# PKU-DAIR/Hetu-Galvatron

Measured on NVIDIA H100. Metric: tokens/sec Llama-3.2-1B-shaped ZeRO-2 training step at 1/2/4/8 H100 vs ref CPU, higher is better.
Workload: dtype bf16

## Files before the change

### hetu-galvatron_b200/csrc/bg_gemm.cu

```cuda
#include <stdlib.h>

#include "bg_ctx.cuh"

using namespace bg;

namespace {

constexpr int BLOCK_M = 128, BLOCK_N = 128, BLOCK_K = 64, WGMMA_K = 16;
constexpr int kStages = 5;
constexpr int kABytes = BLOCK_M * BLOCK_K * 2, kBBytes = BLOCK_N * BLOCK_K * 2, kStageBytes = kABytes + kBBytes;
constexpr int kStoreCols = 64;
constexpr int kStoreBytes = BLOCK_M * kStoreCols * 2;
constexpr int kNumStoreBufs = 2;
constexpr int kSmemBytes = kStages * kStageBytes + kNumStoreBufs * kStoreBytes + 1024  + 256 ;
constexpr int kEpiThreads = 256, kThreads = kEpiThreads + 32;
constexpr int kProducerWarp = kEpiThreads / 32;
constexpr int kMaxRegs = 136;
constexpr int kWgOffset = 8192;
constexpr int kGroupM = 16;
static_assert(kSmemBytes <= 227 * 1024, "H100: at most 227 KiB of shared memory per block");
static_assert(kThreads * kMaxRegs + 3 * 128 * 64 <= 65536, "a GEMM CTA and three slim collective CTAs share an SM's registers");
static_assert(kSmemBytes + 1024 + 3 * 1024 <= 228 * 1024, "a GEMM CTA and three slim collective CTAs share an SM's shared memory");

enum Layout { kTN = 0, kNN = 1, kNT = 2 };

__device__ __forceinline__ uint32_t smem_u32(const void* p) { return (uint32_t)__cvta_generic_to_shared(p); }

__device__ __forceinline__ void mbar_init(uint32_t bar, uint32_t count) {
    asm volatile("mbarrier.init.shared::cta.b64 [%0], %1;" ::"r"(bar), "r"(count));
}
__device__ __forceinline__ void mbar_wait(uint32_t bar, uint32_t parity) {
    asm volatile(
        "{\n\t.reg .pred p;\n\t"
        "WAIT_%=:\n\t"
        "mbarrier.try_wait.parity.shared::cta.b64 p, [%0], %1;\n\t"
        "@p bra DONE_%=;\n\t"
        "bra WAIT_%=;\n\t"
        "DONE_%=:\n\t}" ::"r"(bar), "r"(parity) : "memory");
}
__device__ __forceinline__ void mbar_arrive(uint32_t bar) {
    asm volatile("mbarrier.arrive.shared::cta.b64 _, [%0];" ::"r"(bar) : "memory");
}
__device__ __forceinline__ void mbar_expect_tx(uint32_t bar, uint32_t bytes) {
    asm volatile("mbarrier.arrive.expect_tx.shared::cta.b64 _, [%0], %1;" ::"r"(bar), "r"(bytes) : "memory");
}
__device__ __forceinline__ void tma_load_2d(uint32_t dst, const CUtensorMap* map, uint32_t bar, int c0, int c1) {
    asm volatile("cp.async.bulk.tensor.2d.shared::cluster.global.mbarrier::complete_tx::bytes [%0], [%1, {%3, %4}], [%2];"
                 ::"r"(dst), "l"(map), "r"(bar), "r"(c0), "r"(c1) : "memory");
}
__device__ __forceinline__ void tma_store_2d(const CUtensorMap* map, uint32_t src, int c0, int c1) {
    asm volatile("cp.async.bulk.tensor.2d.global.shared::cta.bulk_group [%0, {%2, %3}], [%1];"
                 ::"l"(map), "r"(src), "r"(c0), "r"(c1) : "memory");
}
__device__ __forceinline__ void tma_store_commit() { asm volatile("cp.async.bulk.commit_group;" ::: "memory"); }
template <int N>
__device__ __forceinline__ void tma_store_wait_read() { asm volatile("cp.async.bulk.wait_group.read %0;" ::"n"(N) : "memory"); }
template <int N>
__device__ __forceinline__ void tma_store_wait_all() { asm volatile("cp.async.bulk.wait_group %0;" ::"n"(N) : "memory"); }
__device__ __forceinline__ void fence_proxy_async() { asm volatile("fence.proxy.async.shared::cta;" ::: "memory"); }
__device__ __forceinline__ void epi_bar_sync() { asm volatile("bar.sync 1, %0;" ::"n"(kEpiThreads) : "memory"); }
__device__ __forceinline__ bool elect_one() {
    uint32_t pred;
    asm volatile("{\n\t.reg .pred p;\n\telect.sync _|p, 0xffffffff;\n\tselp.u32 %0, 1, 0, p;\n\t}" : "=r"(pred));
    return pred != 0;
}

__device__ __forceinline__ void wgmma_fence() { asm volatile("wgmma.fence.sync.aligned;" ::: "memory"); }
__device__ __forceinline__ void wgmma_commit() { asm volatile("wgmma.commit_group.sync.aligned;" ::: "memory"); }
template <int N>
__device__ __forceinline__ void wgmma_wait() { asm volatile("wgmma.wait_group.sync.aligned %0;" ::"n"(N) : "memory"); }
__device__ __forceinline__ void fence_acc(float* d) {
#pragma unroll
    for (int i = 0; i < BLOCK_N / 2; ++i) asm volatile("" : "+f"(d[i])::"memory");
}

template <int kTransA, int kTransB>
__device__ __forceinline__ void wgmma_m64n128(float* d, uint64_t desc_a, uint64_t desc_b, uint32_t accumulate) {
    asm volatile(
        "{\n\t.reg .pred p;\n\t"
        "setp.ne.b32 p, %66, 0;\n\t"
        "wgmma.mma_async.sync.aligned.m64n128k16.f32.bf16.bf16 "
        "{%0, %1, %2, %3, %4, %5, %6, %7, %8, %9, %10, %11, %12, %13, %14, %15, "
        "%16, %17, %18, %19, %20, %21, %22, %23, %24, %25, %26, %27, %28, %29, %30, %31, "
        "%32, %33, %34, %35, %36, %37, %38, %39, %40, %41, %42, %43, %44, %45, %46, %47, "
        "%48, %49, %50, %51, %52, %53, %54, %55, %56, %57, %58, %59, %60, %61, %62, %63}, "
        "%64, %65, p, 1, 1, %67, %68;\n\t}"
        : "+f"(d[0]), "+f"(d[1]), "+f"(d[2]), "+f"(d[3]), "+f"(d[4]), "+f"(d[5]), "+f"(d[6]), "+f"(d[7]),
          "+f"(d[8]), "+f"(d[9]), "+f"(d[10]), "+f"(d[11]), "+f"(d[12]), "+f"(d[13]), "+f"(d[14]), "+f"(d[15]),
          "+f"(d[16]), "+f"(d[17]), "+f"(d[18]), "+f"(d[19]), "+f"(d[20]), "+f"(d[21]), "+f"(d[22]), "+f"(d[23]),
          "+f"(d[24]), "+f"(d[25]), "+f"(d[26]), "+f"(d[27]), "+f"(d[28]), "+f"(d[29]), "+f"(d[30]), "+f"(d[31]),
          "+f"(d[32]), "+f"(d[33]), "+f"(d[34]), "+f"(d[35]), "+f"(d[36]), "+f"(d[37]), "+f"(d[38]), "+f"(d[39]),
          "+f"(d[40]), "+f"(d[41]), "+f"(d[42]), "+f"(d[43]), "+f"(d[44]), "+f"(d[45]), "+f"(d[46]), "+f"(d[47]),
          "+f"(d[48]), "+f"(d[49]), "+f"(d[50]), "+f"(d[51]), "+f"(d[52]), "+f"(d[53]), "+f"(d[54]), "+f"(d[55]),
          "+f"(d[56]), "+f"(d[57]), "+f"(d[58]), "+f"(d[59]), "+f"(d[60]), "+f"(d[61]), "+f"(d[62]), "+f"(d[63])
        : "l"(desc_a), "l"(desc_b), "r"(accumulate), "n"(kTransA), "n"(kTransB));
}

__device__ __forceinline__ uint64_t make_smem_desc(uint32_t smem_addr, uint32_t lbo_bytes, uint32_t sbo_bytes) {
    uint64_t d = 0;
    d |= (uint64_t)((smem_addr >> 4) & 0x3fff);
    d |= (uint64_t)((lbo_bytes >> 4) & 0x3fff) << 16;
    d |= (uint64_t)((sbo_bytes >> 4) & 0x3fff) << 32;
    d |= (uint64_t)1 << 62;
    return d;
}

struct TileCoord { int m, n; };
enum { kPlain = 0, kScatterMode = 1, kGatherMode = 2 };

template <int kMode>
struct FuseParams {};

template <>
struct FuseParams<kPlain> {
    int group_m;
};

__device__ __forceinline__ TileCoord tile_of_virtual(int t, int m_blocks, int n_blocks, int group_m) {
    const int per_group = group_m * n_blocks;
    const int g = t / per_group, first_m = g * group_m;
    const int rows = min(group_m, m_blocks - first_m);
    const int r = t - g * per_group;
    return {first_m + r % rows, r / rows};
}

template <>
struct FuseParams<kScatterMode> {
    CUtensorMap dst[BG_MAX_PEERS];
    uint32_t* flags[BG_MAX_PEERS];
    int p, me, rows_per_rank;
};

template <>
struct FuseParams<kGatherMode> {
    CUtensorMap a_local;
    const uint32_t* flags;
    uint32_t target;
    int p, me, blocks_per_rank;
    unsigned long long timeout_ns;
    int* err;
};

template <int kMode>
__device__ __forceinline__ int map_m(int mv, int m_blocks, const FuseParams<kMode>& fp) {
    if constexpr (kMode == kScatterMode) {
        int m = mv + ((fp.me + 1) % fp.p) * (fp.rows_per_rank / BLOCK_M);
        return m >= m_blocks ? m - m_blocks : m;
    } else if constexpr (kMode == kGatherMode) {
        const int c = mv / fp.p, k = mv - c * fp.p;
        int slot = fp.me + k; if (slot >= fp.p) slot -= fp.p;
        return slot * fp.blocks_per_rank + c;
    } else {
        return mv;
    }
}
template <int kMode>
__device__ __forceinline__ TileCoord tile_of(int t, int m_blocks, int n_blocks, const FuseParams<kMode>& fp) {
    int group_m = kGroupM;
    if constexpr (kMode == kPlain) group_m = fp.group_m;
    TileCoord tc = tile_of_virtual(t, m_blocks, n_blocks, group_m);
    tc.m = map_m<kMode>(tc.m, m_blocks, fp);
    return tc;
}

template <int kLayout, int kMode = kPlain>
__global__ void __maxnreg__(kMaxRegs) gemm_bf16_kernel(const __grid_constant__ CUtensorMap map_a,
                                                                const __grid_constant__ CUtensorMap map_b,
                                                                const __grid_constant__ CUtensorMap map_c,
                                                                const __nv_bfloat16* __restrict__ c_old, int M, int N, int K,
                                                                int accumulate,
                                                                const __grid_constant__ FuseParams<kMode> sp) {
    constexpr bool kScatter = kMode == kScatterMode, kGather = kMode == kGatherMode;
    constexpr bool kAMn = kLayout == kNT, kBMn = kLayout != kTN;
    extern __shared__ uint8_t smem_raw[];
    uint8_t* smem = reinterpret_cast<uint8_t*>((reinterpret_cast<uintptr_t>(smem_raw) + 1023) & ~uintptr_t(1023));
    uint8_t* smem_store = smem + kStages * kStageBytes;
    uint64_t* bars = reinterpret_cast<uint64_t*>(smem_store + kNumStoreBufs * kStoreBytes);
    uint64_t* full_bar = bars;
    uint64_t* empty_bar = bars + kStages;

    const int warp = threadIdx.x >> 5, lane = threadIdx.x & 31;
    const int m_blocks = (M + BLOCK_M - 1) / BLOCK_M, n_blocks = (N + BLOCK_N - 1) / BLOCK_N;
    const int num_tiles = m_blocks * n_blocks, k_blocks = (K + BLOCK_K - 1) / BLOCK_K;

    if constexpr (kScatter) {
        asm volatile("griddepcontrol.launch_dependents;" ::: "memory");
    }
    if (warp == kProducerWarp && lane == 0) {
        asm volatile("prefetch.tensormap [%0];" ::"l"(&map_a) : "memory");
        asm volatile("prefetch.tensormap [%0];" ::"l"(&map_b) : "memory");
        asm volatile("prefetch.tensormap [%0];" ::"l"(&map_c) : "memory");
        for (int i = 0; i < kStages; ++i) { mbar_init(smem_u32(full_bar + i), 1); mbar_init(smem_u32(empty_bar + i), kEpiThreads / 32); }
        asm volatile("fence.mbarrier_init.release.cluster;" ::: "memory");
    }
    __syncthreads();

    if (warp == kProducerWarp) {
        if (elect_one()) {
            int stage = 0; uint32_t phase = 0;
            for (int t = blockIdx.x; t < num_tiles; t += gridDim.x) {
                const TileCoord tc = tile_of<kMode>(t, m_blocks, n_blocks, sp);
                const CUtensorMap* amap = &map_a;
                int a_row = tc.m * BLOCK_M;
                if constexpr (kGather) {
                    const int slot = tc.m / sp.blocks_per_rank, c = tc.m - slot * sp.blocks_per_rank;
                    if (slot == sp.me) {
                        amap = &sp.a_local; a_row = c * BLOCK_M;
                    } else {
                        const uint32_t* f = sp.flags + slot * sp.blocks_per_rank + c;
                        unsigned long long t0 = 0; unsigned spins = 0;
                        while (true) {
                            uint32_t v;
                            asm volatile("ld.acquire.sys.global.u32 %0, [%1];" : "=r"(v) : "l"(f) : "memory");
                            if (v >= sp.target) break;
                            if ((++spins & 0x3ff) == 0) {
                                unsigned long long now = gtimer();
                                if (t0 == 0) t0 = now;
                                else if (now - t0 > sp.timeout_ns) {
                                    if (atomicCAS(sp.err + 1, 0, 4) == 0) { sp.err[2] = (int)blockIdx.x; sp.err[3] = tc.m; sp.err[4] = (int)v; sp.err[5] = (int)sp.target; sp.err[6] = slot; }
                                    *sp.err = BG_ETIMEOUT; __threadfence_system(); __trap();
                                }
                            }
                        }
                        asm volatile("fence.proxy.async.global;" ::: "memory");
                    }
                }
                for (int kb = 0; kb < k_blocks; ++kb) {
                    mbar_wait(smem_u32(empty_bar + stage), phase ^ 1);
                    const uint32_t bar = smem_u32(full_bar + stage);
                    const uint32_t sa = smem_u32(smem + stage * kStageBytes), sb = sa + kABytes;
                    mbar_expect_tx(bar, kStageBytes);
                    if (kAMn) {
#pragma unroll
                        for (int j = 0; j < BLOCK_M / 64; ++j) tma_load_2d(sa + j * (BLOCK_K * 128), &map_a, bar, tc.m * BLOCK_M + j * 64, kb * BLOCK_K);
                    } else {
                        tma_load_2d(sa, amap, bar, kb * BLOCK_K, a_row);
                    }
                    if (kBMn) {
#pragma unroll
                        for (int j = 0; j < BLOCK_N / 64; ++j) tma_load_2d(sb + j * (BLOCK_K * 128), &map_b, bar, tc.n * BLOCK_N + j * 64, kb * BLOCK_K);
                    } else {
                        tma_load_2d(sb, &map_b, bar, kb * BLOCK_K, tc.n * BLOCK_N);
                    }
                    if (++stage == kStages) { stage = 0; phase ^= 1; }
                }
            }
        }
    } else {
        const int wg = warp >> 2;
        const int frag_row = wg * 64 + (warp & 3) * 16 + (lane >> 2);
        const int frag_col = (lane & 3) * 2;
        const bool issuer = threadIdx.x == 0;
        constexpr uint32_t a_lbo = kAMn ? BLOCK_K * 128 : 0, b_lbo = kBMn ? BLOCK_K * 128 : 0;
        constexpr uint32_t a_kstep = kAMn ? WGMMA_K * 128 : WGMMA_K * 2, b_kstep = kBMn ? WGMMA_K * 128 : WGMMA_K * 2;
        float acc[BLOCK_N / 2];
#pragma unroll
        for (int i = 0; i < BLOCK_N / 2; ++i) acc[i] = 0.f;
        int stage = 0; uint32_t phase = 0;
        int buf = 0;
        uint32_t* prev_flag = nullptr;
        for (int t = blockIdx.x; t < num_tiles; t += gridDim.x) {
            const TileCoord tc = tile_of<kMode>(t, m_blocks, n_blocks, sp);
            int prev_stage = 0;
            for (int kb = 0; kb < k_blocks; ++kb) {
                mbar_wait(smem_u32(full_bar + stage), phase);
                const uint32_t sa = smem_u32(smem + stage * kStageBytes) + wg * kWgOffset;
                const uint32_t sb = smem_u32(smem + stage * kStageBytes) + kABytes;
                wgmma_fence();
#pragma unroll
                for (int k = 0; k < BLOCK_K / WGMMA_K; ++k) {
                    const uint64_t da = make_smem_desc(sa + k * a_kstep, a_lbo, 1024);
                    const uint64_t db = make_smem_desc(sb + k * b_kstep, b_lbo, 1024);
                    wgmma_m64n128<kAMn ? 1 : 0, kBMn ? 1 : 0>(acc, da, db, (kb | k) != 0);
                }
                wgmma_commit();
                wgmma_wait<1>();
                if (kb > 0 && lane == 0) mbar_arrive(smem_u32(empty_bar + prev_stage));
                prev_stage = stage;
                if (++stage == kStages) { stage = 0; phase ^= 1; }
            }
            wgmma_wait<0>();
            fence_acc(acc);
            if (lane == 0) mbar_arrive(smem_u32(empty_bar + prev_stage));
#pragma unroll
            for (int c = 0; c < BLOCK_N / kStoreCols; ++c) {
                const int n0 = tc.n * BLOCK_N + c * kStoreCols;
                if (n0 >= N) break;
                float* v = acc + c * (kStoreCols / 2);
                if (accumulate) {
#pragma unroll
                    for (int h = 0; h < 2; ++h) {
                        const long long grow = (long long)tc.m * BLOCK_M + frag_row + 8 * h;
                        if (grow < M) {
#pragma unroll
                            for (int j = 0; j < 8; ++j) {
                                if (n0 + j * 8 < N) {
                                    const float2 o = bf2_to_f2(*reinterpret_cast<const uint32_t*>(c_old + grow * N + n0 + j * 8 + frag_col));
                                    v[j * 4 + 2 * h] += o.x;
                                    v[j * 4 + 2 * h + 1] += o.y;
                                }
                            }
                        }
                    }
                }
                if (issuer) tma_store_wait_read<kNumStoreBufs - 1>();
                epi_bar_sync();
                uint8_t* sbuf = smem_store + buf * kStoreBytes;
#pragma unroll
                for (int h = 0; h < 2; ++h) {
                    const int row = frag_row + 8 * h;
#pragma unroll
                    for (int j = 0; j < 8; ++j)
                        *reinterpret_cast<uint32_t*>(sbuf + row * 128 + ((j ^ (row & 7)) << 4) + frag_col * 2) =
                            f2_to_bf2(v[j * 4 + 2 * h], v[j * 4 + 2 * h + 1]);
                }
                fence_proxy_async();
                epi_bar_sync();
                if (issuer) {
                    if constexpr (kScatter) {
                        const int row0 = tc.m * BLOCK_M, owner = row0 / sp.rows_per_rank;
                        tma_store_2d(&sp.dst[owner], smem_u32(sbuf), n0, sp.me * sp.rows_per_rank + (row0 - owner * sp.rows_per_rank));
                    } else {
                        tma_store_2d(&map_c, smem_u32(sbuf), n0, tc.m * BLOCK_M);
                    }
                    tma_store_commit();
                }
                buf ^= 1;
            }
            if constexpr (kScatter) {
                if (issuer) {
                    if (prev_flag != nullptr) {
                        asm volatile("cp.async.bulk.wait_group %0;" ::"n"(BLOCK_N / kStoreCols) : "memory");
                        __threadfence_system();
                        asm volatile("red.release.sys.global.add.u32 [%0], 1;" ::"l"(prev_flag) : "memory");
                    }
                    const int row0 = tc.m * BLOCK_M, owner = row0 / sp.rows_per_rank;
                    prev_flag = sp.flags[owner] + ((row0 - owner * sp.rows_per_rank) / BLOCK_M) * n_blocks + tc.n;
                }
            }
        }
        if (issuer) {
            tma_store_wait_all<0>();
            if constexpr (kScatter) {
                if (prev_flag != nullptr) {
                    __threadfence_system();
                    asm volatile("red.release.sys.global.add.u32 [%0], 1;" ::"l"(prev_flag) : "memory");
                }
            }
        }
    }
}

typedef CUresult (*EncodeTiledFn)(CUtensorMap*, CUtensorMapDataType, cuuint32_t, void*, const cuuint64_t*, const cuuint64_t*,
                                  const cuuint32_t*, const cuuint32_t*, CUtensorMapInterleave, CUtensorMapSwizzle,
                                  CUtensorMapL2promotion, CUtensorMapFloatOOBfill);

EncodeTiledFn encode_fn() {
    static EncodeTiledFn fn = nullptr;
    static std::once_flag once;
    std::call_once(once, [] {
        void* p = nullptr;
        cudaDriverEntryPointQueryResult q;
        if (cudaGetDriverEntryPoint("cuTensorMapEncodeTiled", &p, cudaEnableDefault, &q) == cudaSuccess && q == cudaDriverEntryPointSuccess)
            fn = (EncodeTiledFn)p;
    });
    return fn;
}

int make_map(CUtensorMap* map, const void* ptr, long long rows, long long cols, int box_cols, int box_rows) {
    EncodeTiledFn fn = encode_fn();
    if (!fn) return fail(BG_ECUDA, "cuTensorMapEncodeTiled entry point not available");
    cuuint64_t dims[2] = {(cuuint64_t)cols, (cuuint64_t)rows};
    cuuint64_t strides[1] = {(cuuint64_t)cols * 2};
    cuuint32_t box[2] = {(cuuint32_t)box_cols, (cuuint32_t)box_rows};
    cuuint32_t estr[2] = {1, 1};
    CUresult r = fn(map, CU_TENSOR_MAP_DATA_TYPE_BFLOAT16, 2, const_cast<void*>(ptr), dims, strides, box, estr,
                    CU_TENSOR_MAP_INTERLEAVE_NONE, CU_TENSOR_MAP_SWIZZLE_128B, CU_TENSOR_MAP_L2_PROMOTION_L2_256B,
                    CU_TENSOR_MAP_FLOAT_OOB_FILL_NONE);
    if (r == CUDA_ERROR_INVALID_CONTEXT) {
        cudaFree(0);
        r = fn(map, CU_TENSOR_MAP_DATA_TYPE_BFLOAT16, 2, const_cast<void*>(ptr), dims, strides, box, estr,
               CU_TENSOR_MAP_INTERLEAVE_NONE, CU_TENSOR_MAP_SWIZZLE_128B, CU_TENSOR_MAP_L2_PROMOTION_L2_256B,
               CU_TENSOR_MAP_FLOAT_OOB_FILL_NONE);
    }
    if (r != CUDA_SUCCESS) return fail(BG_ECUDA, "cuTensorMapEncodeTiled failed (%d) rows=%lld cols=%lld", (int)r, rows, cols);
    return BG_OK;
}

int g_num_sms = 0;

}

int bg_preload_gemm();

static int gemm_setup() {
    if (g_num_sms == 0) {
        int dev = 0;
        BG_CUDA(cudaGetDevice(&dev));
        int sms = 0;
        BG_CUDA(cudaDeviceGetAttribute(&sms, cudaDevAttrMultiProcessorCount, dev));
#define BG_SMEM(K) BG_CUDA(cudaFuncSetAttribute(K, cudaFuncAttributeMaxDynamicSharedMemorySize, kSmemBytes))
        BG_SMEM(gemm_bf16_kernel<kTN>); BG_SMEM(gemm_bf16_kernel<kNN>); BG_SMEM(gemm_bf16_kernel<kNT>);
        BG_SMEM((gemm_bf16_kernel<kTN, kScatterMode>)); BG_SMEM((gemm_bf16_kernel<kNN, kScatterMode>)); BG_SMEM((gemm_bf16_kernel<kNT, kScatterMode>));
        BG_SMEM((gemm_bf16_kernel<kTN, kGatherMode>)); BG_SMEM((gemm_bf16_kernel<kNN, kGatherMode>));
#undef BG_SMEM
        g_num_sms = sms;
    }
    return BG_OK;
}



static int make_ab_maps(CUtensorMap* ma, CUtensorMap* mb, const void* a, const void* b, long long m, long long n, long long k, int layout) {
    int rc = layout == kNT ? make_map(ma, a, k, m, 64, BLOCK_K) : make_map(ma, a, m, k, BLOCK_K, BLOCK_M);
    if (rc) return rc;
    return layout == kTN ? make_map(mb, b, n, k, BLOCK_K, BLOCK_N) : make_map(mb, b, k, n, 64, BLOCK_K);
}

static int gemm_launch(const void* a, const void* b, void* c, const void* addend, long long m, long long n, long long k, int layout, void* stream);

extern "C" int bg_gemm_bf16(const void* a, const void* b, void* c, long long m, long long n, long long k, int layout,
                            int accumulate, void* stream) {
    return gemm_launch(a, b, c, accumulate ? c : nullptr, m, n, k, layout, stream);
}

extern "C" int bg_gemm_bf16_add(const void* a, const void* b, void* c, const void* addend, long long m, long long n, long long k,
                                int layout, void* stream) {
    if (addend == nullptr || (uintptr_t)addend % 16) return fail(BG_EINVAL, "bg_gemm_bf16_add: addend must be a 16-B aligned [M][N] bf16 tensor");
    return gemm_launch(a, b, c, addend, m, n, k, layout, stream);
}

static int gemm_launch(const void* a, const void* b, void* c, const void* addend, long long m, long long n, long long k, int layout, void* stream) {
    const int accumulate = addend != nullptr;
    if (layout < 0 || layout > 2) return fail(BG_EINVAL, "bg_gemm_bf16: layout %d", layout);
    if (m <= 0 || n <= 0 || k <= 0 || m % 8 || n % 8 || k % 8)
        return fail(BG_EINVAL, "bg_gemm_bf16: m,n,k (%lld,%lld,%lld) must be positive multiples of 8", m, n, k);
    if (((uintptr_t)a | (uintptr_t)b | (uintptr_t)c) % 16) return fail(BG_EINVAL, "bg_gemm_bf16: pointers must be 16-B aligned");
    CUtensorMap ma, mb, mc;
    int rc = make_ab_maps(&ma, &mb, a, b, m, n, k, layout);
    if (rc) return rc;
    rc = make_map(&mc, c, m, n, kStoreCols, BLOCK_M);
    if (rc) return rc;
    rc = gemm_setup();
    if (rc) return rc;
    const long long n_blocks = (n + BLOCK_N - 1) / BLOCK_N, tiles = ((m + BLOCK_M - 1) / BLOCK_M) * n_blocks;
    const int grid = (int)(tiles < g_num_sms ? tiles : g_num_sms);
    cudaStream_t st = (cudaStream_t)stream;
    const __nv_bfloat16* c_old = (const __nv_bfloat16*)addend;
    FuseParams<kPlain> plain;
    plain.group_m = n_blocks <= 32 ? 2 : 8;
    if (layout == kTN) gemm_bf16_kernel<kTN><<<grid, kThreads, kSmemBytes, st>>>(ma, mb, mc, c_old, (int)m, (int)n, (int)k, accumulate, plain);
    else if (layout == kNN) gemm_bf16_kernel<kNN><<<grid, kThreads, kSmemBytes, st>>>(ma, mb, mc, c_old, (int)m, (int)n, (int)k, accumulate, plain);
    else gemm_bf16_kernel<kNT><<<grid, kThreads, kSmemBytes, st>>>(ma, mb, mc, c_old, (int)m, (int)n, (int)k, accumulate, plain);
    BG_CHECK_LAUNCH();
    return BG_OK;
}

namespace {

struct Bcast {
    char* out[BG_MAX_PEERS];
    char* mc;
    int on;
};

__device__ __forceinline__ void mm_st_16g(void* mc, const uint4& v) {
    asm volatile("multimem.st.relaxed.sys.global.v4.f32 [%0], {%1,%2,%3,%4};" ::"l"(mc), "f"(__uint_as_float(v.x)),
                 "f"(__uint_as_float(v.y)), "f"(__uint_as_float(v.z)), "f"(__uint_as_float(v.w)) : "memory");
}

__global__ void __launch_bounds__(128, 8) tile_reduce_kernel(const __nv_bfloat16* __restrict__ partial, uint32_t* __restrict__ flags,
                                                          __nv_bfloat16* __restrict__ out, int p, int me, int rows_per_rank, int N,
                                                          int n_blocks, int local_tiles, const __grid_constant__ Bcast bc,
                                                          unsigned long long timeout_ns, int* err) {
    for (int lt = blockIdx.x; lt < local_tiles; lt += gridDim.x) {
        if (threadIdx.x == 0) {
            unsigned long long t0 = 0;
            unsigned spins = 0;
            while (true) {
                uint32_t v;
                asm volatile("ld.acquire.sys.global.u32 %0, [%1];" : "=r"(v) : "l"(flags + lt) : "memory");
                if (v >= (uint32_t)p) break;
                if ((++spins & 0x3ff) == 0) {
                    unsigned long long now = gtimer();
                    if (t0 == 0) t0 = now;
                    else if (now - t0 > timeout_ns / 2) {
                        if (atomicCAS(err + 1, 0, 3) == 0) { err[2] = (int)blockIdx.x; err[3] = lt; err[4] = (int)v; err[5] = p; err[6] = local_tiles; }
                        *err = BG_ETIMEOUT; __threadfence_system(); __trap();
                    }
                }
            }
        }
        __syncthreads();
        const int mb = lt / n_blocks, nb = lt % n_blocks;
        const int row0 = mb * BLOCK_M, col0 = nb * BLOCK_N;
        const int cols = min(BLOCK_N, N - col0), rows = min(BLOCK_M, rows_per_rank - row0);
        const int vec_per_row = cols / 8;
        for (int i = threadIdx.x; i < rows * vec_per_row; i += blockDim.x) {
            const int r = i / vec_per_row, c = i - r * vec_per_row;
            const size_t off = (size_t)(row0 + r) * N + col0 + c * 8;
            uint4 in[BG_MAX_PEERS];
#pragma unroll
            for (int src = 0; src < BG_MAX_PEERS; ++src)
                if (src < p) in[src] = ld16_stream(partial + (size_t)src * rows_per_rank * N + off);
            float acc[8];
#pragma unroll
            for (int e = 0; e < 8; ++e) acc[e] = 0.f;
#pragma unroll
            for (int src = 0; src < BG_MAX_PEERS; ++src)
                if (src < p) {
                    float f[8];
                    unpack8(in[src], f);
#pragma unroll
                    for (int e = 0; e < 8; ++e) acc[e] += f[e];
                }
            const uint4 o = pack8(acc);
            if (bc.on) {
                const size_t goff = ((size_t)me * rows_per_rank * N + off) * 2;
                if (bc.mc != nullptr) {
                    mm_st_16g(bc.mc + goff, o);
                } else {
                    for (int k = 0; k < p; ++k) {
                        int q = me + k; if (q >= p) q -= p;
                        st16(bc.out[q] + goff, o);
                    }
                }
            } else {
                st16(out + off, o);
            }
        }
        __syncthreads();
        if (threadIdx.x == 0) flags[lt] = 0;
    }
    asm volatile("griddepcontrol.wait;" ::: "memory");
}

}

int bg_gemm_scatter_launch(const void* a, const void* b, long long m, long long n, long long k, int layout, int p, int me,
                           void* const* partial_ptrs, uint32_t* const* flag_ptrs, void* out, void* const* bcast_ptrs, char* bcast_mc,
                           unsigned long long timeout_ns, int* err_dev, cudaStream_t st) {
    if (layout < 0 || layout > 2) return fail(BG_EINVAL, "bg_gemm_reduce_scatter: layout %d", layout);
    if (m <= 0 || n <= 0 || k <= 0 || n % 8 || k % 8) return fail(BG_EINVAL, "bg_gemm_reduce_scatter: bad dims");
    if (m % ((long long)p * BLOCK_M)) return fail(BG_EINVAL, "bg_gemm_reduce_scatter: M=%lld must be a multiple of p*%d", m, BLOCK_M);
    const int rows_per_rank = (int)(m / p);
    CUtensorMap ma, mb;
    int rc = make_ab_maps(&ma, &mb, a, b, m, n, k, layout);
    if (rc) return rc;
    FuseParams<kScatterMode> sp;
    sp.p = p; sp.me = me; sp.rows_per_rank = rows_per_rank;
    for (int i = 0; i < BG_MAX_PEERS; ++i) {
        sp.flags[i] = i < p ? flag_ptrs[i] : nullptr;
        if (i < p) { rc = make_map(&sp.dst[i], partial_ptrs[i], (long long)p * rows_per_rank, n, kStoreCols, BLOCK_M); if (rc) return rc; }
        else sp.dst[i] = sp.dst[0];
    }
    rc = gemm_setup();
    if (rc) return rc;
    const int m_blocks = (int)((m + BLOCK_M - 1) / BLOCK_M), n_blocks = (int)((n + BLOCK_N - 1) / BLOCK_N);
    const long long tiles = (long long)m_blocks * n_blocks;
    const int grid = (int)(tiles < g_num_sms ? tiles : g_num_sms);
    const int local_tiles = (rows_per_rank / BLOCK_M) * n_blocks;
    const CUtensorMap& mc_unused = sp.dst[0];
    if (layout == kTN) gemm_bf16_kernel<kTN, kScatterMode><<<grid, kThreads, kSmemBytes, st>>>(ma, mb, mc_unused, nullptr, (int)m, (int)n, (int)k, 0, sp);
    else if (layout == kNN) gemm_bf16_kernel<kNN, kScatterMode><<<grid, kThreads, kSmemBytes, st>>>(ma, mb, mc_unused, nullptr, (int)m, (int)n, (int)k, 0, sp);
    else gemm_bf16_kernel<kNT, kScatterMode><<<grid, kThreads, kSmemBytes, st>>>(ma, mb, mc_unused, nullptr, (int)m, (int)n, (int)k, 0, sp);
    BG_CHECK_LAUNCH();
    const int rgrid = local_tiles < g_num_sms ? local_tiles : g_num_sms;
    Bcast bc = {};
    if (bcast_ptrs != nullptr) {
        bc.on = 1; bc.mc = bcast_mc;
        for (int i = 0; i < p; ++i) bc.out[i] = (char*)bcast_ptrs[i];
    }
    cudaLaunchConfig_t cfg = {};
    cfg.gridDim = dim3((unsigned)rgrid); cfg.blockDim = dim3(128);
    cudaLaunchAttribute attr[1];
    attr[0].id = cudaLaunchAttributeProgrammaticStreamSerialization;
    attr[0].val.programmaticStreamSerializationAllowed = 1;
    static const bool no_pdl = getenv("HGB_NO_PDL") != nullptr;
    cfg.attrs = attr; cfg.numAttrs = no_pdl ? 0 : 1;
    BG_CUDA(cudaLaunchKernelEx(&cfg, tile_reduce_kernel, (const __nv_bfloat16*)partial_ptrs[me], (uint32_t*)flag_ptrs[me],
                               (__nv_bfloat16*)out, p, me, rows_per_rank, (int)n, n_blocks, local_tiles, bc, timeout_ns, err_dev));
    bg::g_launches.fetch_add(1, std::memory_order_relaxed);
    return BG_OK;
}

int bg_gemm_gather_launch(const void* a_local, const void* a_staged, const void* b, void* c, long long m, long long n, long long k,
                          int layout, int p, int me, const uint32_t* flags, uint32_t target, unsigned long long timeout_ns, int* err_dev,
                          cudaStream_t st) {
    if (layout != kTN && layout != kNN) return fail(BG_EINVAL, "bg_all_gather_gemm: layout %d", layout);
    if (((uintptr_t)a_local | (uintptr_t)a_staged | (uintptr_t)b | (uintptr_t)c) % 16) return fail(BG_EINVAL, "bg_all_gather_gemm: pointers must be 16-B aligned");
    CUtensorMap ma, mb, mc;
    int rc = make_ab_maps(&ma, &mb, a_staged, b, m, n, k, layout);
    if (rc) return rc;
    rc = make_map(&mc, c, m, n, kStoreCols, BLOCK_M);
    if (rc) return rc;
    FuseParams<kGatherMode> gp;
    rc = make_map(&gp.a_local, a_local, m / p, k, BLOCK_K, BLOCK_M);
    if (rc) return rc;
    gp.flags = flags; gp.target = target; gp.p = p; gp.me = me; gp.blocks_per_rank = (int)(m / p / BLOCK_M);
    gp.timeout_ns = timeout_ns; gp.err = err_dev;
    rc = gemm_setup();
    if (rc) return rc;
    const long long tiles = (m / BLOCK_M) * ((n + BLOCK_N - 1) / BLOCK_N);
    const int grid = (int)(tiles < g_num_sms ? tiles : g_num_sms);
    if (layout == kTN) gemm_bf16_kernel<kTN, kGatherMode><<<grid, kThreads, kSmemBytes, st>>>(ma, mb, mc, nullptr, (int)m, (int)n, (int)k, 0, gp);
    else gemm_bf16_kernel<kNN, kGatherMode><<<grid, kThreads, kSmemBytes, st>>>(ma, mb, mc, nullptr, (int)m, (int)n, (int)k, 0, gp);
    BG_CHECK_LAUNCH();
    return BG_OK;
}

int bg_preload_gemm() {
    int rc = gemm_setup();
    if (rc) return rc;
    cudaFuncAttributes attr;
    BG_CUDA(cudaFuncGetAttributes(&attr, reinterpret_cast<const void*>(&tile_reduce_kernel)));
    return BG_OK;
}
```

Baseline: 51740.

## Add 128x256 wide-tile WGMMA path for plain GEMMs with N above 128

Templates the GEMM kernel on tile width and adds a 128x256 variant using m64n256 WGMMA, with 4 stages, a single store buffer and a 168-register cap. Plain GEMMs with N>128 now use the wide tile, which halves B-operand reloads per output and amortizes A loads over twice the columns. The group_m swizzle heuristic also changes. Risks are higher register pressure, fewer pipeline stages, a serialized epilogue store buffer, and fewer tiles, which can leave SMs idle on small GEMMs.

After: 54300 (median of 6 runs). +5.0%, better.

```diff
diff --git a/hetu-galvatron_b200/csrc/bg_gemm.cu b/hetu-galvatron_b200/csrc/bg_gemm.cu
--- a/hetu-galvatron_b200/csrc/bg_gemm.cu
+++ b/hetu-galvatron_b200/csrc/bg_gemm.cu
@@ -7,20 +7,31 @@
 namespace {
 
 constexpr int BLOCK_M = 128, BLOCK_N = 128, BLOCK_K = 64, WGMMA_K = 16;
-constexpr int kStages = 5;
-constexpr int kABytes = BLOCK_M * BLOCK_K * 2, kBBytes = BLOCK_N * BLOCK_K * 2, kStageBytes = kABytes + kBBytes;
+constexpr int WIDE_N = 256;
+constexpr int kABytes = BLOCK_M * BLOCK_K * 2;
 constexpr int kStoreCols = 64;
 constexpr int kStoreBytes = BLOCK_M * kStoreCols * 2;
-constexpr int kNumStoreBufs = 2;
-constexpr int kSmemBytes = kStages * kStageBytes + kNumStoreBufs * kStoreBytes + 1024  + 256 ;
 constexpr int kEpiThreads = 256, kThreads = kEpiThreads + 32;
 constexpr int kProducerWarp = kEpiThreads / 32;
-constexpr int kMaxRegs = 136;
 constexpr int kWgOffset = 8192;
 constexpr int kGroupM = 16;
-static_assert(kSmemBytes <= 227 * 1024, "H100: at most 227 KiB of shared memory per block");
-static_assert(kThreads * kMaxRegs + 3 * 128 * 64 <= 65536, "a GEMM CTA and three slim collective CTAs share an SM's registers");
-static_assert(kSmemBytes + 1024 + 3 * 1024 <= 228 * 1024, "a GEMM CTA and three slim collective CTAs share an SM's shared memory");
+
+template <int kBlockN>
+struct Tile {
+    static constexpr bool kWide = kBlockN == WIDE_N;
+    static constexpr int kStages = kWide ? 4 : 5;
+    static constexpr int kNumStoreBufs = kWide ? 1 : 2;
+    static constexpr int kMaxRegs = kWide ? 168 : 136;
+    static constexpr int kSlimCtas = kWide ? 2 : 3;
+    static constexpr int kBBytes = kBlockN * BLOCK_K * 2, kStageBytes = kABytes + kBBytes;
+    static constexpr int kSmemBytes = kStages * kStageBytes + kNumStoreBufs * kStoreBytes + 1024  + 256 ;
+    static_assert(kBlockN == BLOCK_N || kBlockN == WIDE_N, "tile width 128 or 256");
+    static_assert(kSmemBytes <= 227 * 1024, "H100: at most 227 KiB of shared memory per block");
+    static_assert(kThreads * kMaxRegs + kSlimCtas * 128 * 64 <= 65536, "a GEMM CTA and its slim collective CTAs share an SM's registers");
+    static_assert(kSmemBytes + 1024 + kSlimCtas * 1024 <= 228 * 1024, "a GEMM CTA and its slim collective CTAs share an SM's shared memory");
+};
+template struct Tile<BLOCK_N>;
+template struct Tile<WIDE_N>;
 
 enum Layout { kTN = 0, kNN = 1, kNT = 2 };
 
@@ -69,9 +80,10 @@
 __device__ __forceinline__ void wgmma_commit() { asm volatile("wgmma.commit_group.sync.aligned;" ::: "memory"); }
 template <int N>
 __device__ __forceinline__ void wgmma_wait() { asm volatile("wgmma.wait_group.sync.aligned %0;" ::"n"(N) : "memory"); }
+template <int kNumAcc>
 __device__ __forceinline__ void fence_acc(float* d) {
 #pragma unroll
-    for (int i = 0; i < BLOCK_N / 2; ++i) asm volatile("" : "+f"(d[i])::"memory");
+    for (int i = 0; i < kNumAcc; ++i) asm volatile("" : "+f"(d[i])::"memory");
 }
 
 template <int kTransA, int kTransB>
@@ -96,6 +108,40 @@
         : "l"(desc_a), "l"(desc_b), "r"(accumulate), "n"(kTransA), "n"(kTransB));
 }
 
+template <int kTransA, int kTransB>
+__device__ __forceinline__ void wgmma_m64n256(float* d, uint64_t desc_a, uint64_t desc_b, uint32_t accumulate) {
+    asm volatile(
+        "{\n\t.reg .pred p;\n\t"
+        "setp.ne.b32 p, %130, 0;\n\t"
+        "wgmma.mma_async.sync.aligned.m64n256k16.f32.bf16.bf16 "
+        "{%0, %1, %2, %3, %4, %5, %6, %7, %8, %9, %10, %11, %12, %13, %14, %15, "
+        "%16, %17, %18, %19, %20, %21, %22, %23, %24, %25, %26, %27, %28, %29, %30, %31, "
+        "%32, %33, %34, %35, %36, %37, %38, %39, %40, %41, %42, %43, %44, %45, %46, %47, "
+        "%48, %49, %50, %51, %52, %53, %54, %55, %56, %57, %58, %59, %60, %61, %62, %63, "
+        "%64, %65, %66, %67, %68, %69, %70, %71, %72, %73, %74, %75, %76, %77, %78, %79, "
+        "%80, %81, %82, %83, %84, %85, %86, %87, %88, %89, %90, %91, %92, %93, %94, %95, "
+        "%96, %97, %98, %99, %100, %101, %102, %103, %104, %105, %106, %107, %108, %109, %110, %111, "
+        "%112, %113, %114, %115, %116, %117, %118, %119, %120, %121, %122, %123, %124, %125, %126, %127}, "
+        "%128, %129, p, 1, 1, %131, %132;\n\t}"
+        : "+f"(d[0]), "+f"(d[1]), "+f"(d[2]), "+f"(d[3]), "+f"(d[4]), "+f"(d[5]), "+f"(d[6]), "+f"(d[7]),
+          "+f"(d[8]), "+f"(d[9]), "+f"(d[10]), "+f"(d[11]), "+f"(d[12]), "+f"(d[13]), "+f"(d[14]), "+f"(d[15]),
+          "+f"(d[16]), "+f"(d[17]), "+f"(d[18]), "+f"(d[19]), "+f"(d[20]), "+f"(d[21]), "+f"(d[22]), "+f"(d[23]),
+          "+f"(d[24]), "+f"(d[25]), "+f"(d[26]), "+f"(d[27]), "+f"(d[28]), "+f"(d[29]), "+f"(d[30]), "+f"(d[31]),
+          "+f"(d[32]), "+f"(d[33]), "+f"(d[34]), "+f"(d[35]), "+f"(d[36]), "+f"(d[37]), "+f"(d[38]), "+f"(d[39]),
+          "+f"(d[40]), "+f"(d[41]), "+f"(d[42]), "+f"(d[43]), "+f"(d[44]), "+f"(d[45]), "+f"(d[46]), "+f"(d[47]),
+          "+f"(d[48]), "+f"(d[49]), "+f"(d[50]), "+f"(d[51]), "+f"(d[52]), "+f"(d[53]), "+f"(d[54]), "+f"(d[55]),
+          "+f"(d[56]), "+f"(d[57]), "+f"(d[58]), "+f"(d[59]), "+f"(d[60]), "+f"(d[61]), "+f"(d[62]), "+f"(d[63]),
+          "+f"(d[64]), "+f"(d[65]), "+f"(d[66]), "+f"(d[67]), "+f"(d[68]), "+f"(d[69]), "+f"(d[70]), "+f"(d[71]),
+          "+f"(d[72]), "+f"(d[73]), "+f"(d[74]), "+f"(d[75]), "+f"(d[76]), "+f"(d[77]), "+f"(d[78]), "+f"(d[79]),
+          "+f"(d[80]), "+f"(d[81]), "+f"(d[82]), "+f"(d[83]), "+f"(d[84]), "+f"(d[85]), "+f"(d[86]), "+f"(d[87]),
+          "+f"(d[88]), "+f"(d[89]), "+f"(d[90]), "+f"(d[91]), "+f"(d[92]), "+f"(d[93]), "+f"(d[94]), "+f"(d[95]),
+          "+f"(d[96]), "+f"(d[97]), "+f"(d[98]), "+f"(d[99]), "+f"(d[100]), "+f"(d[101]), "+f"(d[102]), "+f"(d[103]),
+          "+f"(d[104]), "+f"(d[105]), "+f"(d[106]), "+f"(d[107]), "+f"(d[108]), "+f"(d[109]), "+f"(d[110]), "+f"(d[111]),
+          "+f"(d[112]), "+f"(d[113]), "+f"(d[114]), "+f"(d[115]), "+f"(d[116]), "+f"(d[117]), "+f"(d[118]), "+f"(d[119]),
+          "+f"(d[120]), "+f"(d[121]), "+f"(d[122]), "+f"(d[123]), "+f"(d[124]), "+f"(d[125]), "+f"(d[126]), "+f"(d[127])
+        : "l"(desc_a), "l"(desc_b), "r"(accumulate), "n"(kTransA), "n"(kTransB));
+}
+
 __device__ __forceinline__ uint64_t make_smem_desc(uint32_t smem_addr, uint32_t lbo_bytes, uint32_t sbo_bytes) {
     uint64_t d = 0;
     d |= (uint64_t)((smem_addr >> 4) & 0x3fff);
@@ -163,15 +209,18 @@
     return tc;
 }
 
-template <int kLayout, int kMode = kPlain>
-__global__ void __maxnreg__(kMaxRegs) gemm_bf16_kernel(const __grid_constant__ CUtensorMap map_a,
+template <int kLayout, int kMode = kPlain, int kBlockN = BLOCK_N>
+__global__ void __maxnreg__(Tile<kBlockN>::kMaxRegs) gemm_bf16_kernel(const __grid_constant__ CUtensorMap map_a,
                                                                 const __grid_constant__ CUtensorMap map_b,
                                                                 const __grid_constant__ CUtensorMap map_c,
                                                                 const __nv_bfloat16* __restrict__ c_old, int M, int N, int K,
                                                                 int accumulate,
                                                                 const __grid_constant__ FuseParams<kMode> sp) {
+    static_assert(kMode == kPlain || kBlockN == BLOCK_N, "the fused modes wait on peers: they keep the three-slim-CTA tile");
     constexpr bool kScatter = kMode == kScatterMode, kGather = kMode == kGatherMode;
     constexpr bool kAMn = kLayout == kNT, kBMn = kLayout != kTN;
+    constexpr int kStages = Tile<kBlockN>::kStages, kStageBytes = Tile<kBlockN>::kStageBytes;
+    constexpr int kNumStoreBufs = Tile<kBlockN>::kNumStoreBufs;
     extern __shared__ uint8_t smem_raw[];
     uint8_t* smem = reinterpret_cast<uint8_t*>((reinterpret_cast<uintptr_t>(smem_raw) + 1023) & ~uintptr_t(1023));
     uint8_t* smem_store = smem + kStages * kStageBytes;
@@ -180,7 +229,7 @@
     uint64_t* empty_bar = bars + kStages;
 
     const int warp = threadIdx.x >> 5, lane = threadIdx.x & 31;
-    const int m_blocks = (M + BLOCK_M - 1) / BLOCK_M, n_blocks = (N + BLOCK_N - 1) / BLOCK_N;
+    const int m_blocks = (M + BLOCK_M - 1) / BLOCK_M, n_blocks = (N + kBlockN - 1) / kBlockN;
     const int num_tiles = m_blocks * n_blocks, k_blocks = (K + BLOCK_K - 1) / BLOCK_K;
 
     if constexpr (kScatter) {
@@ -238,9 +287,9 @@
                     }
                     if (kBMn) {
 #pragma unroll
-                        for (int j = 0; j < BLOCK_N / 64; ++j) tma_load_2d(sb + j * (BLOCK_K * 128), &map_b, bar, tc.n * BLOCK_N + j * 64, kb * BLOCK_K);
+                        for (int j = 0; j < kBlockN / 64; ++j) tma_load_2d(sb + j * (BLOCK_K * 128), &map_b, bar, tc.n * kBlockN + j * 64, kb * BLOCK_K);
                     } else {
-                        tma_load_2d(sb, &map_b, bar, kb * BLOCK_K, tc.n * BLOCK_N);
+                        tma_load_2d(sb, &map_b, bar, kb * BLOCK_K, tc.n * kBlockN);
                     }
                     if (++stage == kStages) { stage = 0; phase ^= 1; }
                 }
@@ -253,9 +302,9 @@
         const bool issuer = threadIdx.x == 0;
         constexpr uint32_t a_lbo = kAMn ? BLOCK_K * 128 : 0, b_lbo = kBMn ? BLOCK_K * 128 : 0;
         constexpr uint32_t a_kstep = kAMn ? WGMMA_K * 128 : WGMMA_K * 2, b_kstep = kBMn ? WGMMA_K * 128 : WGMMA_K * 2;
-        float acc[BLOCK_N / 2];
-#pragma unroll
-        for (int i = 0; i < BLOCK_N / 2; ++i) acc[i] = 0.f;
+        float acc[kBlockN / 2];
+#pragma unroll
+        for (int i = 0; i < kBlockN / 2; ++i) acc[i] = 0.f;
         int stage = 0; uint32_t phase = 0;
         int buf = 0;
         uint32_t* prev_flag = nullptr;
@@ -271,7 +320,8 @@
                 for (int k = 0; k < BLOCK_K / WGMMA_K; ++k) {
                     const uint64_t da = make_smem_desc(sa + k * a_kstep, a_lbo, 1024);
                     const uint64_t db = make_smem_desc(sb + k * b_kstep, b_lbo, 1024);
-                    wgmma_m64n128<kAMn ? 1 : 0, kBMn ? 1 : 0>(acc, da, db, (kb | k) != 0);
+                    if constexpr (kBlockN == WIDE_N) wgmma_m64n256<kAMn ? 1 : 0, kBMn ? 1 : 0>(acc, da, db, (kb | k) != 0);
+                    else wgmma_m64n128<kAMn ? 1 : 0, kBMn ? 1 : 0>(acc, da, db, (kb | k) != 0);
                 }
                 wgmma_commit();
                 wgmma_wait<1>();
@@ -280,14 +330,30 @@
                 if (++stage == kStages) { stage = 0; phase ^= 1; }
             }
             wgmma_wait<0>();
-            fence_acc(acc);
+            fence_acc<kBlockN / 2>(acc);
             if (lane == 0) mbar_arrive(smem_u32(empty_bar + prev_stage));
 #pragma unroll
-            for (int c = 0; c < BLOCK_N / kStoreCols; ++c) {
-                const int n0 = tc.n * BLOCK_N + c * kStoreCols;
+            for (int c = 0; c < kBlockN / kStoreCols; ++c) {
+                const int n0 = tc.n * kBlockN + c * kStoreCols;
                 if (n0 >= N) break;
                 float* v = acc + c * (kStoreCols / 2);
-                if (accumulate) {
+                if (accumulate && Tile<kBlockN>::kWide) {
+#pragma unroll
+                    for (int h = 0; h < 2; ++h) {
+                        const int grow = tc.m * BLOCK_M + frag_row + 8 * h;
+                        if (grow < M) {
+                            const uint32_t* src = reinterpret_cast<const uint32_t*>(c_old + (long long)grow * N + n0 + frag_col);
+#pragma unroll
+                            for (int j = 0; j < 8; ++j) {
+                                if (n0 + j * 8 < N) {
+                                    const float2 o = bf2_to_f2(src[j * 4]);
+                                    v[j * 4 + 2 * h] += o.x;
+                                    v[j * 4 + 2 * h + 1] += o.y;
+                                }
+                            }
+                        }
+                    }
+                } else if (accumulate) {
 #pragma unroll
                     for (int h = 0; h < 2; ++h) {
                         const long long grow = (long long)tc.m * BLOCK_M + frag_row + 8 * h;
@@ -306,13 +372,25 @@
                 if (issuer) tma_store_wait_read<kNumStoreBufs - 1>();
                 epi_bar_sync();
                 uint8_t* sbuf = smem_store + buf * kStoreBytes;
-#pragma unroll
-                for (int h = 0; h < 2; ++h) {
-                    const int row = frag_row + 8 * h;
-#pragma unroll
-                    for (int j = 0; j < 8; ++j)
-                        *reinterpret_cast<uint32_t*>(sbuf + row * 128 + ((j ^ (row & 7)) << 4) + frag_col * 2) =
-                            f2_to_bf2(v[j * 4 + 2 * h], v[j * 4 + 2 * h + 1]);
+                if constexpr (Tile<kBlockN>::kWide) {
+                    uint32_t srow = smem_u32(sbuf) + frag_row * 128 + ((frag_row & 7) << 4) + frag_col * 2;
+                    asm volatile("" : "+r"(srow));
+#pragma unroll
+                    for (int h = 0; h < 2; ++h) {
+#pragma unroll
+                        for (int j = 0; j < 8; ++j)
+                            asm volatile("st.shared.u32 [%0], %1;" ::"r"((srow + h * 1024) ^ (j << 4)),
+                                         "r"(f2_to_bf2(v[j * 4 + 2 * h], v[j * 4 + 2 * h + 1])) : "memory");
+                    }
+                } else {
+#pragma unroll
+                    for (int h = 0; h < 2; ++h) {
+                        const int row = frag_row + 8 * h;
+#pragma unroll
+                        for (int j = 0; j < 8; ++j)
+                            *reinterpret_cast<uint32_t*>(sbuf + row * 128 + ((j ^ (row & 7)) << 4) + frag_col * 2) =
+                                f2_to_bf2(v[j * 4 + 2 * h], v[j * 4 + 2 * h + 1]);
+                    }
                 }
                 fence_proxy_async();
                 epi_bar_sync();
@@ -325,12 +403,12 @@
                     }
                     tma_store_commit();
                 }
-                buf ^= 1;
+                if constexpr (kNumStoreBufs > 1) buf ^= 1;
             }
             if constexpr (kScatter) {
                 if (issuer) {
                     if (prev_flag != nullptr) {
-                        asm volatile("cp.async.bulk.wait_group %0;" ::"n"(BLOCK_N / kStoreCols) : "memory");
+                        asm volatile("cp.async.bulk.wait_group %0;" ::"n"(kBlockN / kStoreCols) : "memory");
                         __threadfence_system();
                         asm volatile("red.release.sys.global.add.u32 [%0], 1;" ::"l"(prev_flag) : "memory");
                     }
@@ -399,10 +477,13 @@
         BG_CUDA(cudaGetDevice(&dev));
         int sms = 0;
         BG_CUDA(cudaDeviceGetAttribute(&sms, cudaDevAttrMultiProcessorCount, dev));
-#define BG_SMEM(K) BG_CUDA(cudaFuncSetAttribute(K, cudaFuncAttributeMaxDynamicSharedMemorySize, kSmemBytes))
-        BG_SMEM(gemm_bf16_kernel<kTN>); BG_SMEM(gemm_bf16_kernel<kNN>); BG_SMEM(gemm_bf16_kernel<kNT>);
-        BG_SMEM((gemm_bf16_kernel<kTN, kScatterMode>)); BG_SMEM((gemm_bf16_kernel<kNN, kScatterMode>)); BG_SMEM((gemm_bf16_kernel<kNT, kScatterMode>));
-        BG_SMEM((gemm_bf16_kernel<kTN, kGatherMode>)); BG_SMEM((gemm_bf16_kernel<kNN, kGatherMode>));
+#define BG_SMEM(K, W) BG_CUDA(cudaFuncSetAttribute(K, cudaFuncAttributeMaxDynamicSharedMemorySize, Tile<W>::kSmemBytes))
+        BG_SMEM(gemm_bf16_kernel<kTN>, BLOCK_N); BG_SMEM(gemm_bf16_kernel<kNN>, BLOCK_N); BG_SMEM(gemm_bf16_kernel<kNT>, BLOCK_N);
+        BG_SMEM((gemm_bf16_kernel<kTN, kPlain, WIDE_N>), WIDE_N); BG_SMEM((gemm_bf16_kernel<kNN, kPlain, WIDE_N>), WIDE_N);
+        BG_SMEM((gemm_bf16_kernel<kNT, kPlain, WIDE_N>), WIDE_N);
+        BG_SMEM((gemm_bf16_kernel<kTN, kScatterMode>), BLOCK_N); BG_SMEM((gemm_bf16_kernel<kNN, kScatterMode>), BLOCK_N);
+        BG_SMEM((gemm_bf16_kernel<kNT, kScatterMode>), BLOCK_N);
+        BG_SMEM((gemm_bf16_kernel<kTN, kGatherMode>), BLOCK_N); BG_SMEM((gemm_bf16_kernel<kNN, kGatherMode>), BLOCK_N);
 #undef BG_SMEM
         g_num_sms = sms;
     }
@@ -411,10 +492,11 @@
 
 
 
-static int make_ab_maps(CUtensorMap* ma, CUtensorMap* mb, const void* a, const void* b, long long m, long long n, long long k, int layout) {
+static int make_ab_maps(CUtensorMap* ma, CUtensorMap* mb, const void* a, const void* b, long long m, long long n, long long k, int layout,
+                        int block_n = BLOCK_N) {
     int rc = layout == kNT ? make_map(ma, a, k, m, 64, BLOCK_K) : make_map(ma, a, m, k, BLOCK_K, BLOCK_M);
     if (rc) return rc;
-    return layout == kTN ? make_map(mb, b, n, k, BLOCK_K, BLOCK_N) : make_map(mb, b, k, n, 64, BLOCK_K);
+    return layout == kTN ? make_map(mb, b, n, k, BLOCK_K, block_n) : make_map(mb, b, k, n, 64, BLOCK_K);
 }
 
 static int gemm_launch(const void* a, const void* b, void* c, const void* addend, long long m, long long n, long long k, int layout, void* stream);
@@ -430,28 +512,38 @@
     return gemm_launch(a, b, c, addend, m, n, k, layout, stream);
 }
 
+template <int kBlockN>
+static int plain_launch(const void* a, const void* b, void* c, const void* addend, long long m, long long n, long long k, int layout, void* stream);
+
 static int gemm_launch(const void* a, const void* b, void* c, const void* addend, long long m, long long n, long long k, int layout, void* stream) {
-    const int accumulate = addend != nullptr;
     if (layout < 0 || layout > 2) return fail(BG_EINVAL, "bg_gemm_bf16: layout %d", layout);
     if (m <= 0 || n <= 0 || k <= 0 || m % 8 || n % 8 || k % 8)
         return fail(BG_EINVAL, "bg_gemm_bf16: m,n,k (%lld,%lld,%lld) must be positive multiples of 8", m, n, k);
     if (((uintptr_t)a | (uintptr_t)b | (uintptr_t)c) % 16) return fail(BG_EINVAL, "bg_gemm_bf16: pointers must be 16-B aligned");
+    return n > BLOCK_N ? plain_launch<WIDE_N>(a, b, c, addend, m, n, k, layout, stream)
+                       : plain_launch<BLOCK_N>(a, b, c, addend, m, n, k, layout, stream);
+}
+
+template <int kBlockN>
+static int plain_launch(const void* a, const void* b, void* c, const void* addend, long long m, long long n, long long k, int layout, void* stream) {
     CUtensorMap ma, mb, mc;
-    int rc = make_ab_maps(&ma, &mb, a, b, m, n, k, layout);
+    int rc = make_ab_maps(&ma, &mb, a, b, m, n, k, layout, kBlockN);
     if (rc) return rc;
     rc = make_map(&mc, c, m, n, kStoreCols, BLOCK_M);
     if (rc) return rc;
     rc = gemm_setup();
     if (rc) return rc;
-    const long long n_blocks = (n + BLOCK_N - 1) / BLOCK_N, tiles = ((m + BLOCK_M - 1) / BLOCK_M) * n_blocks;
+    const long long n_blocks = (n + kBlockN - 1) / kBlockN, tiles = ((m + BLOCK_M - 1) / BLOCK_M) * n_blocks;
     const int grid = (int)(tiles < g_num_sms ? tiles : g_num_sms);
     cudaStream_t st = (cudaStream_t)stream;
     const __nv_bfloat16* c_old = (const __nv_bfloat16*)addend;
+    const int accumulate = addend != nullptr;
+    constexpr int smem = Tile<kBlockN>::kSmemBytes;
     FuseParams<kPlain> plain;
-    plain.group_m = n_blocks <= 32 ? 2 : 8;
-    if (layout == kTN) gemm_bf16_kernel<kTN><<<grid, kThreads, kSmemBytes, st>>>(ma, mb, mc, c_old, (int)m, (int)n, (int)k, accumulate, plain);
-    else if (layout == kNN) gemm_bf16_kernel<kNN><<<grid, kThreads, kSmemBytes, st>>>(ma, mb, mc, c_old, (int)m, (int)n, (int)k, accumulate, plain);
-    else gemm_bf16_kernel<kNT><<<grid, kThreads, kSmemBytes, st>>>(ma, mb, mc, c_old, (int)m, (int)n, (int)k, accumulate, plain);
+    plain.group_m = n_blocks <= 16 ? 4 : 16;
+    if (layout == kTN) gemm_bf16_kernel<kTN, kPlain, kBlockN><<<grid, kThreads, smem, st>>>(ma, mb, mc, c_old, (int)m, (int)n, (int)k, accumulate, plain);
+    else if (layout == kNN) gemm_bf16_kernel<kNN, kPlain, kBlockN><<<grid, kThreads, smem, st>>>(ma, mb, mc, c_old, (int)m, (int)n, (int)k, accumulate, plain);
+    else gemm_bf16_kernel<kNT, kPlain, kBlockN><<<grid, kThreads, smem, st>>>(ma, mb, mc, c_old, (int)m, (int)n, (int)k, accumulate, plain);
     BG_CHECK_LAUNCH();
     return BG_OK;
 }
@@ -561,9 +653,9 @@
     const int grid = (int)(tiles < g_num_sms ? tiles : g_num_sms);
     const int local_tiles = (rows_per_rank / BLOCK_M) * n_blocks;
     const CUtensorMap& mc_unused = sp.dst[0];
-    if (layout == kTN) gemm_bf16_kernel<kTN, kScatterMode><<<grid, kThreads, kSmemBytes, st>>>(ma, mb, mc_unused, nullptr, (int)m, (int)n, (int)k, 0, sp);
-    else if (layout == kNN) gemm_bf16_kernel<kNN, kScatterMode><<<grid, kThreads, kSmemBytes, st>>>(ma, mb, mc_unused, nullptr, (int)m, (int)n, (int)k, 0, sp);
-    else gemm_bf16_kernel<kNT, kScatterMode><<<grid, kThreads, kSmemBytes, st>>>(ma, mb, mc_unused, nullptr, (int)m, (int)n, (int)k, 0, sp);
+    if (layout == kTN) gemm_bf16_kernel<kTN, kScatterMode><<<grid, kThreads, Tile<BLOCK_N>::kSmemBytes, st>>>(ma, mb, mc_unused, nullptr, (int)m, (int)n, (int)k, 0, sp);
+    else if (layout == kNN) gemm_bf16_kernel<kNN, kScatterMode><<<grid, kThreads, Tile<BLOCK_N>::kSmemBytes, st>>>(ma, mb, mc_unused, nullptr, (int)m, (int)n, (int)k, 0, sp);
+    else gemm_bf16_kernel<kNT, kScatterMode><<<grid, kThreads, Tile<BLOCK_N>::kSmemBytes, st>>>(ma, mb, mc_unused, nullptr, (int)m, (int)n, (int)k, 0, sp);
     BG_CHECK_LAUNCH();
     const int rgrid = local_tiles < g_num_sms ? local_tiles : g_num_sms;
     Bcast bc = {};
@@ -603,8 +695,8 @@
     if (rc) return rc;
     const long long tiles = (m / BLOCK_M) * ((n + BLOCK_N - 1) / BLOCK_N);
     const int grid = (int)(tiles < g_num_sms ? tiles : g_num_sms);
-    if (layout == kTN) gemm_bf16_kernel<kTN, kGatherMode><<<grid, kThreads, kSmemBytes, st>>>(ma, mb, mc, nullptr, (int)m, (int)n, (int)k, 0, gp);
-    else gemm_bf16_kernel<kNN, kGatherMode><<<grid, kThreads, kSmemBytes, st>>>(ma, mb, mc, nullptr, (int)m, (int)n, (int)k, 0, gp);
+    if (layout == kTN) gemm_bf16_kernel<kTN, kGatherMode><<<grid, kThreads, Tile<BLOCK_N>::kSmemBytes, st>>>(ma, mb, mc, nullptr, (int)m, (int)n, (int)k, 0, gp);
+    else gemm_bf16_kernel<kNN, kGatherMode><<<grid, kThreads, Tile<BLOCK_N>::kSmemBytes, st>>>(ma, mb, mc, nullptr, (int)m, (int)n, (int)k, 0, gp);
     BG_CHECK_LAUNCH();
     return BG_OK;
 }
```
